# imaranresearch/LAMMPS-SPHERHARM

Hardware: NVIDIA B200
Metric: contact_pair_evals_per_s (higher is better)
Workload: dtype f64

## Files before the change

lammps-spherharm_b200/csrc/pair_split_kernels.cuh:

```cuda
#pragma once
#include "pair_kernel.cuh"

namespace shgpu {

#define SPLIT_CAP 88
#define SURV_CAP 320
#define CACHE_CAP 384

struct __align__(16) SurvRec {
  double s0, s1, s2;
  int k;
  int flag;
};

struct __align__(16) PdEntry {
  long long off;
  int cnt;
  unsigned short ntrans;
  unsigned short cnt2;
  unsigned int off2;
  unsigned short nin;
  unsigned short in[5];
};
#define PD_INLINE 5

struct __align__(16) PairHot {
  int i, j, n0, n1;
  long long off;
  int img;
  unsigned char shp_i, shp_j, pad0, pad1;
};

struct EvalPlanDev {
  int total_blocks, nshape;
  int blk_start[SH_MAX_SHAPES + 1];
  long long count[SH_MAX_SHAPES];
};

struct SplitScalars {
  unsigned long long pool_count[SH_MAX_SHAPES];
  unsigned long long in_count;
  int nbig;
  int nslow;
  int slow_counter;
  int deep_counter;
};

struct SplitArgs {
  SurvRec *pool;
  unsigned char *pool_flag;
  const long long *pool_base;
  const long long *pool_cap;
  SplitScalars *sc;
  PdEntry *pd;
  int *big_list;
  int *slow_list;
  int *inpool;
  long long in_cap;
};

struct CacheArgs {
  unsigned short *pool;
  PairHot *hot;
  unsigned long long *count;
  long long cap;
  int *overflow;
  const int *invalid;
  int enabled;
  int level;
};

__device__ __forceinline__ float fp32_margin(float t0, float t1, float t2, float ra) {
  const float sc = sqrtf(fmaf(t2, t2, fmaf(t1, t1, t0 * t0))) + ra;
  return 1.9073486e-6f * sc * sc;
}

struct NodeWindow { bool skip; float cosA, xe, se, phie; };

__device__ __forceinline__ NodeWindow make_window(const DevShape &sa, double Rb, const double *x0) {
  NodeWindow w;
  const double e0 = 2.0 * x0[0], e1 = 2.0 * x0[1], e2 = 2.0 * x0[2];
  const double D2 = e0 * e0 + e1 * e1 + e2 * e2, D = sqrt(D2);
  w.skip = D >= (sa.rmax + Rb) * (1.0 + 1e-9);
  w.cosA = -2.0f; w.xe = 1.0f; w.se = 0.0f; w.phie = 0.0f;
  if (!w.skip && D > 1e-9 * (sa.rmax + Rb)) {
    const double q = D2 - Rb * Rb;
    double rc = sa.rmin;
    if (q > 0) rc = fmin(fmax(sqrt(q), sa.rmin), sa.rmax);
    const double g = (rc * rc + q) / (2.0 * rc * D);
    w.cosA = (float)g - 3e-5f;
    if (w.cosA >= 1.0f) w.skip = true;
    w.xe = fminf(1.0f, fmaxf(-1.0f, (float)(e2 / D)));
    w.se = sqrtf(fmaxf(0.0f, 1.0f - w.xe * w.xe));
    w.phie = atan2f((float)e1, (float)e0);
    if (w.phie < 0.0f) w.phie += 6.2831853f;
  }
  return w;
}

__device__ __forceinline__ void classify_row(const DevShape &sa, const NodeWindow &w, int row, int &c0, int &ccount) {
  c0 = 0; ccount = 0;
  const int nph = sa.n_phi;
  if (row >= sa.n_theta) return;
  if (w.cosA <= -1.0f) { ccount = nph; return; }
  const float xa = sa.row_x[row];
  const float sarow = sqrtf(fmaxf(0.0f, 1.0f - xa * xa));
  const float ss = sarow * w.se, xx = xa * w.xe;
  if (xx + ss < w.cosA) return;
  const float cd = (ss > 1e-12f) ? (w.cosA - xx) / ss : -2.0f;
// ... 13 lines not shown
  int face; float ma, uu, vv;
  if (ax >= ay && ax >= az) { face = f0 > 0 ? 0 : 1; ma = ax; uu = f1; vv = f2; }
  else if (ay >= az) { face = f1 > 0 ? 2 : 3; ma = ay; uu = f0; vv = f2; }
  else { face = f2 > 0 ? 4 : 5; ma = az; uu = f0; vv = f1; }
  const float im = __fdividef(1.0f, fmaxf(ma, 1e-30f)), hn = 0.5f * (float)cn;
  const int iu = min(cn - 1, max(0, (int)((uu * im + 1.0f) * hn)));
  const int iv = min(cn - 1, max(0, (int)((vv * im + 1.0f) * hn)));
  return (face * cn + iu) * cn + iv;
}

__device__ __forceinline__ double pose_element(const PairArgs &A, int a, int b, double dd0, double dd1, double dd2, int l) {
  const int st = A.stride;
  if (l < 9) {
    const int r = l / 3, k = l - 3 * r;
    double m = A.Rs[(0 + r) * st + b] * A.Rs[(0 + k) * st + a];
    m = fma(A.Rs[(3 + r) * st + b], A.Rs[(3 + k) * st + a], m);
    m = fma(A.Rs[(6 + r) * st + b], A.Rs[(6 + k) * st + a], m);
    return m;
  } else if (l < 12) {
    const int r = l - 9;
    double tt = A.Rs[(0 + r) * st + b] * dd0;
    tt = fma(A.Rs[(3 + r) * st + b], dd1, tt);
    tt = fma(A.Rs[(6 + r) * st + b], dd2, tt);
    return tt;
  }
  const int r = l - 12;
  double hx = A.Rs[(0 + r) * st + a] * dd0;
  hx = fma(A.Rs[(3 + r) * st + a], dd1, hx);
  hx = fma(A.Rs[(6 + r) * st + a], dd2, hx);
  return -0.5 * hx;
}
__device__ __forceinline__ void pose_to_smem(const PairArgs &A, int a, int b, double dd0, double dd1, double dd2, int lane,
                                             double *pose) {
  __syncwarp();
  if (lane < 15) pose[lane] = pose_element(A, a, b, dd0, dd1, dd2, lane);
  __syncwarp();
}

__device__ __forceinline__ int exact_node_stage(const double *M, const double *t, double p0, double p1, double p2, double rmax2,
                                                double rmin2, const float2 *__restrict__ cube, int cn, int use_bounds,
                                                double &s0, double &s1, double &s2) {
  s0 = fma(M[0], p0, t[0]); s0 = fma(M[1], p1, s0); s0 = fma(M[2], p2, s0);
  s1 = fma(M[3], p0, t[1]); s1 = fma(M[4], p1, s1); s1 = fma(M[5], p2, s1);
  s2 = fma(M[6], p0, t[2]); s2 = fma(M[7], p1, s2); s2 = fma(M[8], p2, s2);
  const double rho2 = fma(s2, s2, fma(s1, s1, s0 * s0));
  if (!(rho2 < rmax2)) return -1;
  if (rho2 <= rmin2) return 2;
  if (!use_bounds) return 0;
  const float2 ul = __ldg(&cube[cube_cell((float)s0, (float)s1, (float)s2, cn)]);
  if (rho2 <= (double)ul.y) return 2;
  return rho2 < (double)ul.x ? 0 : -1;
}

template <int WPB>
__global__ void __launch_bounds__(WPB * 32) pair_cache_build_kernel(PairArgs A, CacheArgs C, const int *list, const int *nlist) {
  __shared__ unsigned short s_buf[WPB][2][CACHE_CAP];
  __shared__ double s_pose[WPB][16];
  const int lane = threadIdx.x & 31, warp = threadIdx.x >> 5;
  const int nwork = list ? *nlist : A.npairs;
  for (int w = blockIdx.x * WPB + warp; w < nwork; w += gridDim.x * WPB) {
  const int p = list ? list[w] : w;
  const int i = A.pair_i[p], j = A.pair_j[p];
  double d[3];
  pair_separation(A, p, i, j, d);
  const int shp_i = A.shape[i], shp_j = A.shape[j];
  double *pose = s_pose[warp];
  int cnt0 = 0, cnt1 = 0;
  bool over = false;
  for (int dir = 0; dir < 2 && !over; dir++) {
    const int a = dir ? j : i, b = dir ? i : j;
    const DevShape &sa = A.shapes[dir ? shp_j : shp_i];
    const DevShape &sb = A.shapes[dir ? shp_i : shp_j];
    const double sgn = dir ? -1.0 : 1.0;
    pose_to_smem(A, a, b, sgn * d[0], sgn * d[1], sgn * d[2], lane, pose);
    const double *M = pose, *t = pose + 9, *x0 = pose + 12;
    const double delta = sb.cache_delta[C.level], Rb = sb.rmax + delta;
    const NodeWindow w = make_window(sa, Rb, x0);
    const float4 *__restrict__ pf = sa.pf4;
    const float *__restrict__ cube = sb.cube_w2[C.level];
    const int cn = sb.cube_n, nph = sa.n_phi, nth = sa.n_theta;
    const float fM0 = (float)M[0], fM1 = (float)M[1], fM2 = (float)M[2], fM3 = (float)M[3], fM4 = (float)M[4],
                fM5 = (float)M[5], fM6 = (float)M[6], fM7 = (float)M[7], fM8 = (float)M[8];
    const float ft0 = (float)t[0], ft1 = (float)t[1], ft2 = (float)t[2];
    const float eps = fp32_margin(ft0, ft1, ft2, (float)sa.rmax);
    const float fR2 = (float)(Rb * Rb) + eps;
    const float fin = (float)((sb.rmin + 2.0 * delta) * (sb.rmin + 2.0 * delta)) + eps;
    unsigned short *buf = s_buf[warp][dir];
    int n = 0;
    if (!w.skip) {
      for (int rb = 0; rb < nth && !over; rb += 32) {
        int c0, ccount;
        classify_row(sa, w, rb + lane, c0, ccount);
        unsigned rows = __ballot_sync(0xffffffffu, ccount > 0);
        while (rows && !over) {
          const int rl = __ffs(rows) - 1;
          rows &= rows - 1;
          const int rc0 = __shfl_sync(0xffffffffu, c0, rl), rcount = __shfl_sync(0xffffffffu, ccount, rl);
          const int rowbase = (rb + rl) * nph;
          for (int cb = 0; cb < rcount; cb += 32) {
            const int cc = cb + lane;
            bool pass = false;
            int k = 0;
            if (cc < rcount) {
              int col = rc0 + cc;
              if (col >= nph) col -= nph;
              k = rowbase + col;
              const float4 q = __ldg(&pf[k]);
              const float f0 = fmaf(fM2, q.z, fmaf(fM1, q.y, fmaf(fM0, q.x, ft0)));
              const float f1 = fmaf(fM5, q.z, fmaf(fM4, q.y, fmaf(fM3, q.x, ft1)));
              const float f2 = fmaf(fM8, q.z, fmaf(fM7, q.y, fmaf(fM6, q.x, ft2)));
              const float r2 = fmaf(f2, f2, fmaf(f1, f1, f0 * f0));
              if (r2 < fR2) pass = (r2 < fin) || (r2 < __ldg(&cube[cube_cell(f0, f1, f2, cn)]) + eps);
            }
            const unsigned pm = __ballot_sync(0xffffffffu, pass);
            if (pm) {
              const int nnew = __popc(pm);
              if (n + nnew > CACHE_CAP) { over = true; break; }
              if (pass) buf[n + __popc(pm & ((1u << lane) - 1u))] = (unsigned short)k;
              n += nnew;
            }
          }
        }
      }
    }
    if (dir) cnt1 = n; else cnt0 = n;
    __syncwarp();
  }
  const int ntot = cnt0 + cnt1;
  long long off = 0;
  if (lane == 0 && !over && ntot > 0) off = (long long)atomicAdd(C.count, (unsigned long long)ntot);
  off = __shfl_sync(0xffffffffu, off, 0);
  if (!over && ntot > 0) {
    if (off + ntot <= C.cap) {
      for (int r = lane; r < cnt0; r += 32) C.pool[off + r] = s_buf[warp][0][r];
      for (int r = lane; r < cnt1; r += 32) C.pool[off + cnt0 + r] = s_buf[warp][1][r];
    } else { if (lane == 0) *C.overflow = 1; over = true; }
  }
  if (lane == 0) {
    PairHot hrec;
    hrec.i = i; hrec.j = j; hrec.n0 = over ? -1 : cnt0; hrec.n1 = over ? -1 : cnt1; hrec.off = off; hrec.img = A.pair_img[p];
    hrec.shp_i = (unsigned char)shp_i; hrec.shp_j = (unsigned char)shp_j; hrec.pad0 = 0; hrec.pad1 = 0;
    C.hot[p] = hrec;
  }
  __syncwarp();
  }
}

__global__ void cache_remap_kernel(PairArgs A, const int *old_half_off, const int *old_pair_j, int old_nown, const PairHot *old_hot,
                                   const unsigned short *old_pool, CacheArgs C, int *fresh_list, int *nfresh, const int *amap) {
  const int p = blockIdx.x * blockDim.x + threadIdx.x;
  const int lane = threadIdx.x & 31;
  int ntot = 0, q = -1;
  PairHot hrec;
  hrec.i = hrec.j = 0; hrec.n0 = hrec.n1 = 0; hrec.off = 0; hrec.img = 0; hrec.shp_i = hrec.shp_j = 0; hrec.pad0 = hrec.pad1 = 0;
  if (p < A.npairs) {
    const int i = A.pair_i[p], j = A.pair_j[p], img = A.pair_img[p];
    const int oi = amap ? amap[i] : i, oj = amap ? amap[j] : j;
    if (oi >= 0 && oj >= 0 && oi < old_nown && oi < oj)
      for (int e = old_half_off[oi]; e < old_half_off[oi + 1]; e++)
        if (old_pair_j[e] == oj) { q = e; break; }
    if (q >= 0) {
      hrec = old_hot[q];
      if (hrec.n0 < 0 || hrec.img != img || hrec.i != oi || hrec.j != oj) q = -1;
      hrec.i = i; hrec.j = j;
    }
    if (q >= 0) ntot = hrec.n0 + hrec.n1;
    else fresh_list[atomicAdd(nfresh, 1)] = p;
  }
  int pre = ntot;
#pragma unroll
  for (int o = 1; o < 32; o <<= 1) { const int t = __shfl_up_sync(0xffffffffu, pre, o); if (lane >= o) pre += t; }
  const int wtot = __shfl_sync(0xffffffffu, pre, 31);
  long long base = 0;
  if (lane == 31 && wtot > 0) base = (long long)atomicAdd(C.count, (unsigned long long)wtot);
  base = __shfl_sync(0xffffffffu, base, 31);
  if (q >= 0) {
    const long long off = base + (pre - ntot);
    if (off + ntot <= C.cap) {
      const unsigned short *src = old_pool + hrec.off;
      for (int r = 0; r < ntot; r++) C.pool[off + r] = src[r];
      hrec.off = off;
    } else { *C.overflow = 1; hrec.n0 = -1; hrec.n1 = -1; hrec.off = 0; }
    C.hot[p] = hrec;
  }
}

__device__ __forceinline__ void store_pd(PdEntry *dst, long long off, int cnt, int ntrans, int nin, const unsigned short *in,
                                         unsigned int off2 = 0, int cnt2 = 0) {
  PdEntry e;
  e.off = off; e.cnt = cnt; e.ntrans = (unsigned short)ntrans; e.nin = (unsigned short)nin; e.off2 = off2; e.cnt2 = (unsigned short)cnt2;
#pragma unroll
  for (int q = 0; q < PD_INLINE; q++) e.in[q] = (in && q < nin) ? in[q] : (unsigned short)0;
  *dst = e;
}

struct ShapeLite {
  const float4 *pf4; const float2 *cube_ul; const double *px, *py, *pz;
  int cube_n, pad_;
  double rmax, rmax2, rmin2;
};
struct ShapeLiteTable { ShapeLite s[SH_MAX_SHAPES]; };

template <int WPB, int LPP>
__global__ void __launch_bounds__(WPB * 32, 32 / WPB) pair_cull_cached_kernel(PairArgs A, SplitArgs S, CacheArgs C, int use_bounds,
                                                                              const __grid_constant__ ShapeLiteTable T) {
  constexpr int PPW = 32 / LPP, U = 2;
  constexpr unsigned FULLSUB = LPP == 32 ? 0xffffffffu : ((1u << LPP) - 1u);
  __shared__ double s_dpose[WPB][PPW][2][12];
  __shared__ float s_fpose[WPB][PPW][2][12];
  __shared__ unsigned short s_surv[WPB][PPW][SURV_CAP];
  __shared__ signed char s_flag[WPB][PPW][SURV_CAP];
  __shared__ unsigned short s_in[WPB][PPW][2][8];
  const int lane = threadIdx.x & 31, warp = threadIdx.x >> 5;
  const int sub = lane / LPP, sl = lane % LPP, shift = sub * LPP;
  const int p = (blockIdx.x * WPB + warp) * PPW + sub;
  if (*C.invalid) return;
  const bool inrange = p < A.npairs;
  PairHot hot;
  hot.i = hot.j = 0; hot.n0 = hot.n1 = 0; hot.off = 0; hot.img = 21; hot.shp_i = hot.shp_j = 0;
  if (inrange) {
    const int4 *hp = reinterpret_cast<const int4 *>(C.hot + p);
    const int4 h0 = __ldg(hp), h1 = __ldg(hp + 1);
    hot.i = h0.x; hot.j = h0.y; hot.n0 = h0.z; hot.n1 = h0.w;
    hot.off = (long long)(((unsigned long long)(unsigned)h1.y << 32) | (unsigned)h1.x);
    hot.img = h1.z; hot.shp_i = (unsigned char)(h1.w & 255); hot.shp_j = (unsigned char)((h1.w >> 8) & 255);
  }
  if (inrange && hot.n0 < 0 && sl == 0) S.slow_list[atomicAdd(&S.sc->nslow, 1)] = p;
  const bool cached = inrange && hot.n0 >= 0;
  const int n0 = cached ? hot.n0 : 0, n1 = cached ? hot.n1 : 0, ntot = n0 + n1;
  if (cached && ntot == 0 && sl < 2) store_pd(&S.pd[2 * p + sl], 0, 0, 0, 0, nullptr);
  const int maxtot = __reduce_max_sync(0xffffffffu, ntot);
  if (maxtot == 0) return;
  const bool work = ntot > 0;
  const int i = hot.i, j = hot.j, shp_i = hot.shp_i, shp_j = hot.shp_j;
  const ShapeLite &si = T.s[shp_i], &sj = T.s[shp_j];
  if (work) {
    const int st = A.stride;
    double d[3];
#pragma unroll
    for (int k = 0; k < 3; k++) {
      double dk = A.c[k * st + i] - A.c[k * st + j];
      const int n = ((hot.img >> (2 * k)) & 3) - 1;
      if (n != 0) dk = dk - A.boxlen[k] * (double)n;
      d[k] = dk;
    }
    if (sl < 15) {
      const int half = sl >= 12, l = half ? sl - 3 : sl;
      const double sgn = half ? -1.0 : 1.0;
      const double val = pose_element(A, half ? j : i, half ? i : j, sgn * d[0], sgn * d[1], sgn * d[2], l);
      s_dpose[warp][sub][half][l] = val;
      s_fpose[warp][sub][half][l] = (float)val;
      if (sl < 9) {
        const int r = sl / 3, k = sl - 3 * r;
        s_dpose[warp][sub][1][3 * k + r] = val;
        s_fpose[warp][sub][1][3 * k + r] = (float)val;
      }
    }
  }
  __syncwarp();
  const float4 *__restrict__ pf_i = si.pf4, *__restrict__ pf_j = sj.pf4;
  const float2 *__restrict__ cube_i = si.cube_ul, *__restrict__ cube_j = sj.cube_ul;
  const int cn_i = si.cube_n, cn_j = sj.cube_n;
  const float eps0 = fp32_margin(s_fpose[warp][sub][0][9], s_fpose[warp][sub][0][10], s_fpose[warp][sub][0][11], (float)si.rmax);
  const float eps1 = fp32_margin(s_fpose[warp][sub][1][9], s_fpose[warp][sub][1][10], s_fpose[warp][sub][1][11], (float)sj.rmax);
  const float fR20 = (float)sj.rmax2 + eps0, fR21 = (float)si.rmax2 + eps1;
  const unsigned short *__restrict__ cl = C.pool + hot.off;
  unsigned short *surv = s_surv[warp][sub];
  signed char *sflag = s_flag[warp][sub];
  int nsurv = 0, ns0 = 0;
  bool big = false;
  for (int base = 0; base < maxtot; base += LPP * U) {
    int k[U];
    float4 q[U];
    bool pass[U];
#pragma unroll
    for (int u = 0; u < U; u++) {
      const int g = base + LPP * u + sl;
      k[u] = (work && !big && g < ntot) ? (int)__ldg(&cl[g]) : -1;
    }
#pragma unroll
    for (int u = 0; u < U; u++) {
      const int dirc = (base + LPP * u + sl) >= n0;
      q[u] = k[u] >= 0 ? __ldg(&(dirc ? pf_j : pf_i)[k[u]]) : make_float4(0.f, 0.f, 0.f, 0.f);
// ... 504 lines not shown
```

lammps-spherharm_b200/csrc/shgpu_api.cu:

```cuda
#include <cuda_runtime.h>

#include <algorithm>
#include <cmath>
#include <cstdio>
#include <cstring>
#include <string>
#include <vector>

#include "../../include/shgpu.h"
#include "devbuf.h"
#include "dd_types.h"
#include "neighbor_kernels.cuh"
#include "pair_kernel.cuh"
#include "pair_warp_kernel.cuh"
#include "pair_split_kernels.cuh"
#include "shape_tables.h"
#include "step_kernels.cuh"
#include "atom_stress_kernels.cuh"

using namespace shgpu;

namespace {

struct ShapeDev {
// ... 10 lines not shown

struct sh_ctx {
  std::string err;
  int device = 0, sm_count = 148;
  cudaStream_t stream = nullptr;
  double lo[3] = {-1e30, -1e30, -1e30}, hi[3] = {1e30, 1e30, 1e30};
  int periodic[3] = {0, 0, 0};
  bool box_set = false;
  int n_theta = 32, n_phi = 64;
  std::vector<ShapeTables> shapes;
  std::vector<ShapeDev> shape_dev;
  std::vector<DevShape> shape_host_view;
  DevBuf<DevShape> d_shapes;
  bool shapes_dirty = true;
  int total_terms = 0;
  std::vector<double> pk, pm;
  std::vector<double> pgn, pgt, pmu;
  bool dissip = false;
  DevBuf<double> d_pk, d_pm, d_pgn, d_pgt, d_pmu, stress_part;
  bool coeff_dirty = true;
  WallSet walls{};
  double g[3] = {0, 0, 0}, skin = 0.0, dt = 1e-4, gamma_lin = 0.0, gamma_rot = 0.0;
  int neigh_every = 1, neigh_check = 1;
  int64_t n = 0, nghost = 0;
  int stride = 0;
  DevBuf<double> x, v, q, L, f, tq, c, Rs, c0, wallf, ewall, ke;
  DevBuf<int> shape;
  std::vector<int64_t> tag;
  DevBuf<long long> d_tag;
  bool tags_host_valid = true;
  DevBuf<double> gf;
  double time = 0.0;
  DdCtx dd;
  int *h_lagflag = nullptr;
  cudaEvent_t ev_lag[2] = {nullptr, nullptr};
  int lag_slot = 0; bool lag_pending = false, lag_mode = true, lag_pred_valid = false;
  bool cache_sync_ranks = false;
  int64_t step_index = 0, cache_build_step = -10;
  double cache_time = 0.0;
  bool step_trace = false;
  std::vector<cudaEvent_t> ev_step;
  std::vector<float> step_ms;
  std::vector<int> step_flags, step_flags_last;
  DevBuf<int> cell_of, cell_count, cell_start, cell_fill, cell_atoms, tile_sum, cnt_full, cnt_half, nbr_off, half_off,
      nbr_j, pair_i, pair_j, pair_eij, pair_eji, pair_img, scalars;
  DevBuf<double> bbox, slot, pres, stage;
  DevBuf<SurvRec> pool;
  DevBuf<unsigned char> pool_flag;
  DevBuf<long long> pool_base, pool_cap;
  DevBuf<PdEntry> pd;
  DevBuf<PairHot> cache_hot[2];
  DevBuf<SplitScalars> split_sc;
  DevBuf<EvalPlanDev> eval_plan;
  DevBuf<int> big_list, slow_list, split_flags;
  DevBuf<int> inpool;
  long long h_in_cap = 0;
  std::vector<long long> h_pool_cap;
  unsigned long long *h_pool_count = nullptr;
  SplitScalars *h_split_sc = nullptr;
  int *h_cache_invalid = nullptr;
  cudaEvent_t ev_sc = nullptr;
  bool sc_pending = false;
  int sc_nshape = 0;
  double sec_eval = 0, sec_cull = 0, sec_reduce = 0, sec_deep = 0, sec_cache = 0; int64_t eval_launches = 0;
  std::vector<int> ev2_kind;
  int64_t big_pairs = 0, slow_pairs = 0, pool_grows = 0, cache_builds = 0;
  int cache_level = 0, cache_level_pin = -1;
  int64_t cache_age = 0;
  bool cache_exhausted = false;
  int cube_n = 0;
  int reduce_occ = 0;
  int eval_pts = 0, eval_occ = 0, eval_mode = 0;
  long long last_records = 0;
  DevBuf<unsigned short> cache_pool[2];
  DevBuf<int> old_half_off, old_pair_j, fresh_list;
  int old_nown = 0, cache_cur = 0;
  DevBuf<double> old_c, old_cc0, old_cq0;
  DevBuf<long long> old_tag;
  DevBuf<int> ghost_hash, amap;
  int old_n = 0, old_stride = 0, ghost_hash_size = 0;
  bool carry = false;
  int64_t cache_remaps = 0, atoms_epoch = 0, cache_epoch = -1;
  DevBuf<unsigned long long> cache_count;
  long long cache_cap = 0;
  int cache_state = 0;
  DevBuf<double> cc0, cq0, drift;
  bool eval_pending = false;
  DevBuf<unsigned long long> counters;
  int npairs = 0, nentries = 0, nrows = 0;
  int slot_stride = 0, pres_stride = 0;
  int *h_pinned = nullptr;
  bool forces_valid = false, list_valid = false;
  int64_t steps_since_build = 0;
  int64_t neighbor_builds = 0, kernel_launches = 0;
  std::vector<cudaEvent_t> ev, ev2;
  size_t ev_used = 0, ev2_used = 0;
  double sec_pair = 0, sec_neigh = 0, sec_comm = 0, sec_other = 0, sec_run_last = 0, sec_run_total = 0;
  cudaEvent_t run_e0 = nullptr, run_e1 = nullptr;
  int64_t pair_launches = 0;
  DevBuf<double> as_vir, as_kin, as_en, as_send, as_recv;
  DevBuf<int> as_cnt, as_epair;
  int tune_threads = 0, tune_ctas_per_sm = 0, tune_variant = 0, tune_cull_wpb = 0, tune_cull_lpp = 0;
};

namespace {

int fail(sh_ctx *h, const std::string &m) { h->err = m; return -1; }
// ... 271 lines not shown
    return launch_pair_warp<16, true>(h, P, cps, max_grid);
  }
  if (tw == 256) return launch_pair_warp<8, false>(h, P, cps, max_grid);
  return launch_pair_warp<16, false>(h, P, cps, max_grid);
}

template <int WPB, int PTS, int MINB>
int launch_eval(sh_ctx *h, const SplitArgs &S, int maxT) {
  const size_t smem = (size_t)maxT * 24 + 32;
  auto kern = pair_eval_kernel<WPB, PTS, MINB>;
  CU(cudaFuncSetAttribute(kern, cudaFuncAttributeMaxDynamicSharedMemorySize, (int)std::max<size_t>(smem, 48 * 1024)));
  int occ = 0;
  CU(cudaOccupancyMaxActiveBlocksPerMultiprocessor(&occ, kern, WPB * 32, smem));
  if (occ < 1) return fail(h, "pair_eval_kernel does not fit on an SM");
  const int rpb = WPB * 32 * PTS;
  eval_plan_kernel<<<1, 32, 0, h->stream>>>(S, (int)h->shapes.size(), rpb, h->eval_plan.p);
  const int chunked = h->eval_mode == 2;
  int grid = occ * h->sm_count;
  if (!chunked) {
    long long est = h->last_records > 0 ? h->last_records + h->last_records / 16 : 0;
    if (est == 0) for (long long c : h->h_pool_cap) est += c;
    grid = (int)std::max<long long>(grid, std::min<long long>(est / rpb + (long long)h->shapes.size() + 1, 1 << 22));
  }
  kern<<<grid, WPB * 32, smem, h->stream>>>(h->d_shapes.p, S, h->eval_plan.p, h->counters.p, chunked);
  h->kernel_launches += 2;
  return 0;
}

int absorb_split_feedback(sh_ctx *h) {
  if (!h->sc_pending) return 0;
  CU(cudaEventSynchronize(h->ev_sc));
  h->sc_pending = false;
  const SplitScalars &sc = *h->h_split_sc;
  h->big_pairs += sc.nbig; h->slow_pairs += sc.nslow;
  const int ns = std::min<int>(h->sc_nshape, (int)h->h_pool_cap.size());
  for (int s = 0; s < ns; s++)
    if ((long long)sc.pool_count[s] > h->h_pool_cap[s] * 9 / 10) {
      h->h_pool_cap[s] = (long long)(sc.pool_count[s] * 3 / 2) + 4096;
      h->pool_grows++;
    }
  if ((long long)sc.in_count > h->h_in_cap * 9 / 10) { h->h_in_cap = (long long)(sc.in_count * 3 / 2) + 4096; h->pool_grows++; }
  h->last_records = 0;
  for (int s = 0; s < ns; s++) h->last_records += (long long)std::min<unsigned long long>(sc.pool_count[s], (unsigned long long)h->h_pool_cap[s]);
  if (!h->cache_sync_ranks && (h->h_cache_invalid[0] != 0 || h->h_cache_invalid[1] != 0) && h->cache_state != CACHE_INVALID) { h->cache_state = CACHE_INVALID; h->cache_exhausted = true; }
  return 0;
}

int run_split_pipeline(sh_ctx *h, PairArgs &P) {
  const int ns = (int)h->shapes.size(), np = P.npairs;
  constexpr int WPB = 8;
  int rc;
  if ((rc = absorb_split_feedback(h))) return rc;
  try {
    h->pd.ensure((size_t)2 * np + 2); h->big_list.ensure(np + 1); h->slow_list.ensure(np + 1);
    h->pool_base.ensure(SH_MAX_SHAPES); h->pool_cap.ensure(SH_MAX_SHAPES); h->split_sc.ensure(1); h->eval_plan.ensure(1); h->split_flags.ensure(4);
  } catch (std::string &e) { return fail(h, e); }
  if (!h->h_pool_count) {
    CU(cudaMallocHost(&h->h_pool_count, 8 * sizeof(unsigned long long)));
    CU(cudaMallocHost(&h->h_split_sc, sizeof(SplitScalars)));
    CU(cudaMallocHost(&h->h_cache_invalid, 2 * sizeof(int)));
    CU(cudaEventCreateWithFlags(&h->ev_sc, cudaEventDisableTiming));
  }
  if ((int)h->h_pool_cap.size() != ns) {
    h->h_pool_cap.assign(ns, std::max<long long>(4096, (long long)np * 24 / std::max(1, ns) * 2));
  }
  auto tick = [&](int kind) -> int { return ev_tick(h, kind); };
  auto tock = [&]() { ev_tock(h); };
  const int use_bounds = (h->tune_variant & 2) ? 0 : 1;
  CacheArgs C;
  C.enabled = (h->tune_variant & (8 | 2)) ? 0 : 1;
  C.invalid = h->scalars.p + 3;
  if (C.enabled) {
    const int cur = h->cache_cur;
    try { h->cache_hot[cur].ensure((size_t)np + 2); h->cache_count.ensure(2); h->fresh_list.ensure((size_t)np + 2); }
    catch (std::string &e) { return fail(h, e); }
    double pc[3];
    for (int d = 0; d < 3; d++) pc[d] = (h->hi[d] < 1e29 && h->lo[d] > -1e29) ? 0.5 * (h->lo[d] + h->hi[d]) : 0.0;
    auto check_validity = [&]() -> int {
      double dmin = 1e300;
      for (auto &sh : h->shapes) dmin = std::min(dmin, sh.cache_delta[h->cache_level]);
      double rmaxg = 0;
      for (auto &sh : h->shapes) rmaxg = std::max(rmaxg, sh.rmax);
      const double rpair = 2.0 * rmaxg + 2.0 * h->skin;
      CU(cudaMemsetAsync(h->drift.p, 0, CACHE_FIT_N * sizeof(double), h->stream));
      cache_drift_kernel<<<cdiv(h->n, 256), 256, 0, h->stream>>>(view_all(h), pc[0], pc[1], pc[2], h->drift.p);
      cache_fit_solve_kernel<<<1, 32, 0, h->stream>>>(h->drift.p, h->drift.p + 32);
      cache_check_kernel<<<cdiv(h->n, 256), 256, 0, h->stream>>>(view_all(h), h->d_shapes.p, h->cache_level, 0.5 * dmin, h->drift.p + 32,
                                                                 pc[0], pc[1], pc[2], rpair, h->scalars.p + 3);
      h->kernel_launches += 3;
      return 0;
    };
    if (h->cache_state == CACHE_REMAP && h->cache_level + 1 < SH_CACHE_LEVELS && !(h->tune_variant & 32)) {
      const int nxt = 1 - cur;
      try { h->cache_hot[nxt].ensure((size_t)np + 2); h->cache_pool[nxt].ensure((size_t)h->cache_cap + 64); }
      catch (std::string &e) { return fail(h, e); }
      const int *amap = nullptr;
      if (h->carry) {
        try { h->amap.ensure((size_t)h->n + 2); } catch (std::string &e) { return fail(h, e); }
        const int nstay = h->dd.last_nstay, nown = (int)(h->n - h->nghost);
        CU(cudaMemsetAsync(h->drift.p + 64, 0, CACHE_FIT_N * sizeof(double), h->stream));
        const double le_doff = h->dd.le_rate * h->dd.glen[1] * (h->time - h->cache_time);
        dd_cache_map_kernel<<<cdiv(h->n, 256), 256, 0, h->stream>>>(view_all(h), h->d_tag.p, nown, nstay, h->dd.order.p, h->old_tag.p, h->old_c.p,
                                                                    h->old_stride, h->old_nown, h->old_n, h->ghost_hash.p, h->ghost_hash_size,
                                                                    0.25 * h->dd.G.rc * h->dd.G.rc, h->old_cc0.p, h->old_cq0.p, h->amap.p, h->dd.glen[1], le_doff,
                                                                    pc[0], pc[1], pc[2], h->drift.p + 64);
        cache_fit_solve_kernel<<<1, 32, 0, h->stream>>>(h->drift.p + 64, h->drift.p + 96);
        dd_cache_new_atoms_kernel<<<cdiv(h->n, 256), 256, 0, h->stream>>>(view_all(h), h->amap.p, h->drift.p + 96, pc[0], pc[1], pc[2]);
// ... 11 lines not shown
                                                                h->cache_pool[cur].p, C, h->fresh_list.p, h->split_flags.p + 3, amap);
      pair_cache_build_kernel<4><<<std::max(1, std::min(cdiv(np, 4), h->sm_count * 8)), 4 * 32, 0, h->stream>>>(P, C, h->fresh_list.p, h->split_flags.p + 3);
      tock();
      h->kernel_launches += 2;
      h->cache_cur = nxt; h->cache_state = CACHE_VALID; h->cache_remaps++;
    } else if (h->cache_state != CACHE_VALID) {
      if (h->cache_level_pin >= 0) h->cache_level = h->cache_level_pin;
      else if (h->cache_exhausted) {
        if (h->cache_age < 40 && h->cache_level < 1) h->cache_level++;
        else if (h->cache_age > 400 && h->cache_level > 0) h->cache_level--;
      }
      h->cache_exhausted = false;
      if (h->cache_cap < (long long)np * 48) h->cache_cap = (long long)np * 48;
      if (tick(4)) return -2;
      for (int attempt = 0;; attempt++) {
        if (attempt > 6) return fail(h, "candidate cache kept overflowing");
        try { h->cache_pool[cur].ensure((size_t)h->cache_cap + 64); } catch (std::string &e) { return fail(h, e); }
        CU(cudaMemsetAsync(h->cache_count.p, 0, 2 * sizeof(unsigned long long), h->stream));
        CU(cudaMemsetAsync(h->split_flags.p + 2, 0, sizeof(int), h->stream));
        C.pool = h->cache_pool[cur].p; C.hot = h->cache_hot[cur].p; C.count = h->cache_count.p;
        C.cap = h->cache_cap; C.overflow = h->split_flags.p + 2; C.level = h->cache_level;
        pair_cache_build_kernel<4><<<cdiv(np, 4), 4 * 32, 0, h->stream>>>(P, C, nullptr, nullptr);
        h->kernel_launches++;
        CU(cudaMemcpyAsync(h->h_pool_count, h->cache_count.p, sizeof(unsigned long long), cudaMemcpyDeviceToHost, h->stream));
        CU(cudaMemcpyAsync(h->h_pool_count + 1, h->split_flags.p + 2, sizeof(int), cudaMemcpyDeviceToHost, h->stream));
        CU(cudaStreamSynchronize(h->stream));
        if (*reinterpret_cast<const int *>(h->h_pool_count + 1) == 0) break;
        h->cache_cap = (long long)(h->h_pool_count[0] * 3 / 2) + 4096;
      }
      cache_origin_kernel<<<cdiv(h->n, 256), 256, 0, h->stream>>>(view_all(h));
      CU(cudaMemsetAsync(h->scalars.p + 3, 0, 2 * sizeof(int), h->stream));
      tock();
      h->kernel_launches++;
      h->cache_state = CACHE_VALID; h->cache_builds++; h->cache_age = 0; h->cache_epoch = h->atoms_epoch; h->cache_build_step = h->step_index;
      h->cache_time = h->time;
    } else {
      if ((rc = check_validity())) return rc;
    }
    h->cache_age++;
  }
  C.pool = h->cache_pool[h->cache_cur].p; C.hot = h->cache_hot[h->cache_cur].p; C.count = h->cache_count.p;
  C.cap = h->cache_cap; C.overflow = h->split_flags.p + 2; C.level = h->cache_level;
  std::vector<long long> base(ns);
  long long tot = 0;
  for (int s2 = 0; s2 < ns; s2++) { base[s2] = tot; tot += h->h_pool_cap[s2]; }
  if (h->h_in_cap < (long long)np * 2 + 4096) h->h_in_cap = (long long)np * 2 + 4096;
  if (h->h_in_cap > 0xfffffff0LL) h->h_in_cap = 0xfffffff0LL;
  try { h->pool.ensure((size_t)tot + 64); h->pool_flag.ensure((size_t)tot + 64); h->inpool.ensure((size_t)h->h_in_cap + 64); } catch (std::string &e) { return fail(h, e); }
  CU(cudaMemcpyAsync(h->pool_base.p, base.data(), ns * sizeof(long long), cudaMemcpyHostToDevice, h->stream));
  CU(cudaMemcpyAsync(h->pool_cap.p, h->h_pool_cap.data(), ns * sizeof(long long), cudaMemcpyHostToDevice, h->stream));
  CU(cudaMemsetAsync(h->split_sc.p, 0, sizeof(SplitScalars), h->stream));
  SplitArgs S;
  S.pool = h->pool.p; S.pool_flag = h->pool_flag.p; S.pool_base = h->pool_base.p; S.pool_cap = h->pool_cap.p; S.sc = h->split_sc.p;
  S.pd = h->pd.p; S.big_list = h->big_list.p; S.slow_list = h->slow_list.p; S.inpool = h->inpool.p; S.in_cap = h->h_in_cap;
  if (tick(0)) return -2;
  if (C.enabled) {
    const int cw = h->tune_cull_wpb > 0 ? h->tune_cull_wpb : 1;
    const int ppw = h->tune_cull_lpp == 32 ? 1 : 2;
    const int grid = cdiv(np, cw * ppw);
    ShapeLiteTable T{};
    for (int s2 = 0; s2 < ns && s2 < SH_MAX_SHAPES; s2++) {
      const DevShape &v = h->shape_host_view[s2];
      T.s[s2].pf4 = v.pf4; T.s[s2].cube_ul = v.cube_ul; T.s[s2].px = v.px; T.s[s2].py = v.py; T.s[s2].pz = v.pz;
      T.s[s2].cube_n = v.cube_n; T.s[s2].rmax = v.rmax; T.s[s2].rmax2 = v.rmax2; T.s[s2].rmin2 = v.rmin2;
    }
#define LAUNCH_CULL(W, L) pair_cull_cached_kernel<W, L><<<grid, W * 32, 0, h->stream>>>(P, S, C, use_bounds, T)
    if (ppw == 1) { if (cw == 1) LAUNCH_CULL(1, 32); else if (cw == 2) LAUNCH_CULL(2, 32); else if (cw == 8) LAUNCH_CULL(8, 32); else LAUNCH_CULL(4, 32); }
    else { if (cw == 1) LAUNCH_CULL(1, 16); else if (cw == 2) LAUNCH_CULL(2, 16); else if (cw == 8) LAUNCH_CULL(8, 16); else LAUNCH_CULL(4, 16); }
#undef LAUNCH_CULL
    h->kernel_launches++;
  }
  {
    constexpr int WW = 2;
    const int grid = std::max(1, std::min(cdiv(np, WW), h->sm_count * 16));
    pair_cull_window_kernel<WW><<<grid, WW * 32, 0, h->stream>>>(P, S, C, use_bounds);
    h->kernel_launches++;
  }
  tock();
  int maxT = 1;
  for (int s2 = 0; s2 < ns; s2++) maxT = std::max(maxT, h->shape_host_view[s2].nterms4 + 4);
  if (tick(1)) return -2;
  if (h->eval_pts == 2) rc = h->eval_occ == 3 ? launch_eval<WPB, 2, 3>(h, S, maxT) : launch_eval<WPB, 2, 4>(h, S, maxT);
  else rc = launch_eval<WPB, 4, 2>(h, S, maxT);
  if (rc) return rc;
  tock();
  h->eval_launches++;
  if (tick(2)) return -2;
  if (h->reduce_occ == 4) pair_reduce_kernel<4><<<cdiv(np, 128), 128, 0, h->stream>>>(P, S);
  else if (h->reduce_occ == 8) pair_reduce_kernel<8><<<cdiv(np, 128), 128, 0, h->stream>>>(P, S);
  else pair_reduce_kernel<6><<<cdiv(np, 128), 128, 0, h->stream>>>(P, S);
  tock();
  h->kernel_launches++;
  {
    PairArgs Pb = P;
    Pb.pair_list = h->big_list.p; Pb.npairs = np; Pb.npairs_dev = &h->split_sc.p->nbig; Pb.work_counter = &h->split_sc.p->deep_counter;
    if (tick(3)) return -2;
    rc = launch_fused(h, Pb, h->sm_count);
    if (rc) return rc;
    tock();
    h->kernel_launches++;
  }
  CU(cudaMemcpyAsync(h->h_split_sc, h->split_sc.p, sizeof(SplitScalars), cudaMemcpyDeviceToHost, h->stream));
  CU(cudaMemcpyAsync(h->h_cache_invalid, h->scalars.p + 3, 2 * sizeof(int), cudaMemcpyDeviceToHost, h->stream));
  CU(cudaEventRecord(h->ev_sc, h->stream));
  h->sc_pending = true; h->sc_nshape = ns;
  return 0;
}

int compute_forces_device(sh_ctx *h) {
// ... 123 lines not shown
extern "C" {

int sh_version(void) { return 100; }

int sh_create(sh_ctx **out, int device_id) {
  if (!out) return -1;
  *out = nullptr;
  int ndev = 0;
  if (cudaGetDeviceCount(&ndev) != cudaSuccess || ndev == 0) return -3;
  if (device_id < 0 || device_id >= ndev) return -4;
  sh_ctx *h = new sh_ctx();
  h->device = device_id;
  if (cudaSetDevice(device_id) != cudaSuccess) { delete h; return -5; }
  cudaDeviceProp prop;
  cudaGetDeviceProperties(&prop, device_id);
  h->sm_count = prop.multiProcessorCount;
  if (cudaStreamCreateWithFlags(&h->stream, cudaStreamNonBlocking) != cudaSuccess) { delete h; return -6; }
  h->pk.assign(SH_MAX_SHAPES * SH_MAX_SHAPES, 1.0);
  h->pm.assign(SH_MAX_SHAPES * SH_MAX_SHAPES, 1.0);
  h->pgn.assign(SH_MAX_SHAPES * SH_MAX_SHAPES, 0.0); h->pgt.assign(SH_MAX_SHAPES * SH_MAX_SHAPES, 0.0); h->pmu.assign(SH_MAX_SHAPES * SH_MAX_SHAPES, 0.0);
  try {
    h->scalars.ensure(16); h->bbox.ensure(8); h->counters.ensure(16); h->drift.ensure(128);
  } catch (std::string &) { delete h; return -7; }
  cudaMemset(h->scalars.p, 0, 16 * sizeof(int));
  cudaMemset(h->counters.p, 0, 16 * sizeof(unsigned long long));
  cudaMallocHost(&h->h_pinned, 64);
  cudaMallocHost(&h->h_lagflag, 16 * sizeof(int));
  std::memset(h->h_lagflag, 0, 16 * sizeof(int));
  cudaMallocHost(&h->dd.h_int, 256 * sizeof(int));
  for (auto &e : h->ev_lag) cudaEventCreateWithFlags(&e, cudaEventDisableTiming);
  cudaEventCreate(&h->run_e0); cudaEventCreate(&h->run_e1);
  h->ev.resize(2048); h->ev2.resize(4096); h->ev2_kind.resize(2048);
  for (auto &e : h->ev) cudaEventCreate(&e);
  for (auto &e : h->ev2) cudaEventCreate(&e);
  *out = h;
  return 0;
}

int sh_destroy(sh_ctx *h) {
  if (!h) return 0;
  cudaSetDevice(h->device);
  cudaStreamSynchronize(h->stream);
  for (auto &d : h->shape_dev) { d.Ap.release(); d.ab.release(); d.node.release(); d.row_x.release(); d.cube.release(); d.pf4.release(); for (auto &w : d.cubew) w.release(); }
  h->d_shapes.release(); h->d_pk.release(); h->d_pm.release(); h->d_pgn.release(); h->d_pgt.release(); h->d_pmu.release(); h->stress_part.release();
  DevBuf<double> *db[] = {&h->x, &h->v, &h->q, &h->L, &h->f, &h->tq, &h->c, &h->Rs, &h->c0, &h->wallf, &h->ewall, &h->ke, &h->bbox, &h->slot, &h->pres};
  for (auto *b : db) b->release();
  DevBuf<int> *ib[] = {&h->shape, &h->cell_of, &h->cell_count, &h->cell_start, &h->cell_fill, &h->cell_atoms, &h->tile_sum, &h->cnt_full,
                       &h->cnt_half, &h->nbr_off, &h->half_off, &h->nbr_j, &h->pair_i, &h->pair_j, &h->pair_eij, &h->pair_eji, &h->pair_img, &h->scalars};
  for (auto *b : ib) b->release();
  h->counters.release();
  h->as_vir.release(); h->as_kin.release(); h->as_en.release(); h->as_send.release(); h->as_recv.release(); h->as_cnt.release(); h->as_epair.release();
  for (auto &e : h->ev) cudaEventDestroy(e);
  for (auto &e : h->ev2) cudaEventDestroy(e);
  h->pool.release(); h->pool_flag.release(); h->pool_base.release(); h->pool_cap.release(); h->split_sc.release(); h->eval_plan.release(); h->slow_list.release();
  h->pd.release(); h->big_list.release(); h->split_flags.release(); h->inpool.release();
  for (int k = 0; k < 2; k++) { h->cache_hot[k].release(); h->cache_pool[k].release(); }
  h->old_c.release(); h->old_cc0.release(); h->old_cq0.release(); h->old_tag.release(); h->ghost_hash.release(); h->amap.release();
  h->old_half_off.release(); h->old_pair_j.release(); h->fresh_list.release(); h->cache_count.release(); h->cc0.release(); h->cq0.release(); h->drift.release();
  if (h->h_pool_count) { cudaFreeHost(h->h_pool_count); cudaFreeHost(h->h_split_sc); cudaFreeHost(h->h_cache_invalid); cudaEventDestroy(h->ev_sc); }
  if (h->h_pinned) cudaFreeHost(h->h_pinned);
  if (h->h_lagflag) cudaFreeHost(h->h_lagflag);
  if (h->dd.h_int) cudaFreeHost(h->dd.h_int);
  for (auto &e : h->ev_lag) if (e) cudaEventDestroy(e);
  for (auto &e : h->ev_step) cudaEventDestroy(e);
  dd_peer_release(h);
  if (h->dd.peer.d_err) cudaFree(h->dd.peer.d_err);
  h->dd.peer.d_off.release();
  if (h->dd.comm && h->dd.nccl) h->dd.nccl->CommDestroy(h->dd.comm);
  {
    DdCtx &D = h->dd;
    DevBuf<int> *ib2[] = {&D.flag, &D.pos, &D.order, &D.d_int, &D.send_idx, &D.send_slot, &D.shape2};
    for (auto *b : ib2) b->release();
    DevBuf<double> *db2[] = {&D.sendbuf, &D.recvbuf, &D.x2, &D.v2, &D.q2, &D.L2, &h->gf};
    for (auto *b : db2) b->release();
    D.tag2.release(); h->d_tag.release();
  }
  h->stage.release();
  cudaEventDestroy(h->run_e0); cudaEventDestroy(h->run_e1);
  cudaStreamDestroy(h->stream);
  delete h;
  return 0;
}

const char *sh_last_error(const sh_ctx *h) { return h ? h->err.c_str() : "null handle"; }

int sh_set_box(sh_ctx *h, const double lo[3], const double hi[3], const int periodic[3]) {
  for (int d = 0; d < 3; d++) if (!(hi[d] > lo[d])) return fail(h, "box: hi <= lo");
  for (int d = 0; d < 3; d++) { h->lo[d] = lo[d]; h->hi[d] = hi[d]; h->periodic[d] = periodic[d] != 0; }
  for (int d = 0; d < 3; d++) { h->dd.glo[d] = lo[d]; h->dd.ghi[d] = hi[d]; h->dd.gper[d] = periodic[d] != 0; }
  h->dd.geometry_ok = false; h->dd.borders_ok = false;
  h->box_set = true; h->forces_valid = false; h->list_valid = false;
  return 0;
}

int sh_set_quadrature(sh_ctx *h, int n_theta, int n_phi) {
  if (!h->shapes.empty()) return fail(h, "set_quadrature must precede add_shape");
  if (n_theta < 2 || n_phi < 4) return fail(h, "quadrature too small");
  if ((long)n_theta * n_phi > 65535) return fail(h, "quadrature has more than 65535 nodes");
  h->n_theta = n_theta; h->n_phi = n_phi;
  return 0;
}

int sh_add_shape(sh_ctx *h, int lmax, const double *a_lm, const double *b_lm, double density, int *shape_id_out) try {
  if ((int)h->shapes.size() >= SH_MAX_SHAPES) return fail(h, "too many shapes");
  ShapeTables t;
  std::string e = build_shape_tables(lmax, a_lm, b_lm, density, h->n_theta, h->n_phi, t, h->cube_n);
  if (!e.empty()) return fail(h, e);
// ... 882 lines not shown
```

Baseline: 497.2 million.

## Flatten cache-build row loop into packed lane work and warp-cooperative pool copy

The cache-build kernel used to walk each candidate row separately, which left lanes idle on short rows. It now prefix-sums row counts across the warp and maps a flat index onto (row, column) with a binary search over shuffles. Two 32-wide chunks are processed per iteration so loads can overlap. The hot-record migration now copies old pool entries with the whole warp per record instead of one serial loop per lane, at the cost of extra shuffles for index decoding.

```diff
diff --git a/lammps-spherharm_b200/csrc/pair_split_kernels.cuh b/lammps-spherharm_b200/csrc/pair_split_kernels.cuh
--- a/lammps-spherharm_b200/csrc/pair_split_kernels.cuh
+++ b/lammps-spherharm_b200/csrc/pair_split_kernels.cuh
@@ -174,6 +174,7 @@
   return rho2 < (double)ul.x ? 0 : -1;
 }
 
+#define CB_U 2
 template <int WPB>
 __global__ void __launch_bounds__(WPB * 32) pair_cache_build_kernel(PairArgs A, CacheArgs C, const int *list, const int *nlist) {
   __shared__ unsigned short s_buf[WPB][2][CACHE_CAP];
@@ -213,33 +214,48 @@
       for (int rb = 0; rb < nth && !over; rb += 32) {
         int c0, ccount;
         classify_row(sa, w, rb + lane, c0, ccount);
-        unsigned rows = __ballot_sync(0xffffffffu, ccount > 0);
-        while (rows && !over) {
-          const int rl = __ffs(rows) - 1;
-          rows &= rows - 1;
-          const int rc0 = __shfl_sync(0xffffffffu, c0, rl), rcount = __shfl_sync(0xffffffffu, ccount, rl);
-          const int rowbase = (rb + rl) * nph;
-          for (int cb = 0; cb < rcount; cb += 32) {
-            const int cc = cb + lane;
-            bool pass = false;
-            int k = 0;
-            if (cc < rcount) {
-              int col = rc0 + cc;
-              if (col >= nph) col -= nph;
-              k = rowbase + col;
-              const float4 q = __ldg(&pf[k]);
-              const float f0 = fmaf(fM2, q.z, fmaf(fM1, q.y, fmaf(fM0, q.x, ft0)));
-              const float f1 = fmaf(fM5, q.z, fmaf(fM4, q.y, fmaf(fM3, q.x, ft1)));
-              const float f2 = fmaf(fM8, q.z, fmaf(fM7, q.y, fmaf(fM6, q.x, ft2)));
-              const float r2 = fmaf(f2, f2, fmaf(f1, f1, f0 * f0));
-              if (r2 < fR2) pass = (r2 < fin) || (r2 < __ldg(&cube[cube_cell(f0, f1, f2, cn)]) + eps);
-            }
-            const unsigned pm = __ballot_sync(0xffffffffu, pass);
-            if (pm) {
+        int incl = ccount;
+#pragma unroll
+        for (int o = 1; o < 32; o <<= 1) { const int t = __shfl_up_sync(0xffffffffu, incl, o); if (lane >= o) incl += t; }
+        const int excl = incl - ccount, total = __shfl_sync(0xffffffffu, incl, 31);
+        for (int fb = 0; fb < total && !over; fb += 32 * CB_U) {
+          int k[CB_U];
+          bool valid[CB_U], pass[CB_U];
+#pragma unroll
+          for (int u = 0; u < CB_U; u++) {
+            const int f = fb + 32 * u + lane;
+            int r = 0;
+#pragma unroll
+            for (int step = 16; step > 0; step >>= 1)
+              if (__shfl_sync(0xffffffffu, incl, r + step - 1) <= f) r += step;
+            const int rc0 = __shfl_sync(0xffffffffu, c0, r), rex = __shfl_sync(0xffffffffu, excl, r);
+            int col = rc0 + (f - rex);
+            if (col >= nph) col -= nph;
+            valid[u] = f < total;
+            k[u] = valid[u] ? (rb + r) * nph + col : 0;
+          }
+          float4 q[CB_U];
+#pragma unroll
+          for (int u = 0; u < CB_U; u++) q[u] = valid[u] ? __ldg(&pf[k[u]]) : make_float4(0.f, 0.f, 0.f, 0.f);
+#pragma unroll
+          for (int u = 0; u < CB_U; u++) {
+            const float f0 = fmaf(fM2, q[u].z, fmaf(fM1, q[u].y, fmaf(fM0, q[u].x, ft0)));
+            const float f1 = fmaf(fM5, q[u].z, fmaf(fM4, q[u].y, fmaf(fM3, q[u].x, ft1)));
+            const float f2 = fmaf(fM8, q[u].z, fmaf(fM7, q[u].y, fmaf(fM6, q[u].x, ft2)));
+            const float r2 = fmaf(f2, f2, fmaf(f1, f1, f0 * f0));
+            pass[u] = false;
+            if (valid[u] && r2 < fR2) pass[u] = (r2 < fin) || (r2 < __ldg(&cube[cube_cell(f0, f1, f2, cn)]) + eps);
+          }
+#pragma unroll
+          for (int u = 0; u < CB_U; u++) {
+            const unsigned pm = __ballot_sync(0xffffffffu, pass[u]);
+            if (pm && !over) {
               const int nnew = __popc(pm);
-              if (n + nnew > CACHE_CAP) { over = true; break; }
-              if (pass) buf[n + __popc(pm & ((1u << lane) - 1u))] = (unsigned short)k;
-              n += nnew;
+              if (n + nnew > CACHE_CAP) over = true;
+              else {
+                if (pass[u]) buf[n + __popc(pm & ((1u << lane) - 1u))] = (unsigned short)k[u];
+                n += nnew;
+              }
             }
           }
         }
@@ -296,14 +312,19 @@
   long long base = 0;
   if (lane == 31 && wtot > 0) base = (long long)atomicAdd(C.count, (unsigned long long)wtot);
   base = __shfl_sync(0xffffffffu, base, 31);
+  bool copy = false;
+  long long src = 0;
   if (q >= 0) {
     const long long off = base + (pre - ntot);
-    if (off + ntot <= C.cap) {
-      const unsigned short *src = old_pool + hrec.off;
-      for (int r = 0; r < ntot; r++) C.pool[off + r] = src[r];
-      hrec.off = off;
-    } else { *C.overflow = 1; hrec.n0 = -1; hrec.n1 = -1; hrec.off = 0; }
+    if (off + ntot <= C.cap) { copy = ntot > 0; src = hrec.off; hrec.off = off; }
+    else { *C.overflow = 1; hrec.n0 = -1; hrec.n1 = -1; hrec.off = 0; }
     C.hot[p] = hrec;
+  }
+  for (unsigned m = __ballot_sync(0xffffffffu, copy); m; m &= m - 1) {
+    const int l = __ffs(m) - 1;
+    const long long s0 = __shfl_sync(0xffffffffu, src, l), d0 = __shfl_sync(0xffffffffu, hrec.off, l);
+    const int n = __shfl_sync(0xffffffffu, ntot, l);
+    for (int r = lane; r < n; r += 32) C.pool[d0 + r] = old_pool[s0 + r];
   }
 }
 
```

Result: no change. 498.6 million, median of 6 (+0.3%).

## Compact cached cull pairs into a worklist before the cull kernel

Applied to the files above, without the earlier changes.

Adds a pre-pass kernel that classifies each pair: slow pairs go to the slow list, zero-count pairs get empty pd entries, and pairs with work are compacted into a cull list via warp ballot plus atomics. The cull kernel then indexes through this list and exits early for warps past the list length, so no warps are spent on empty or slow pairs. It costs an extra launch, an extra pass over the hot records and one indirection, and the grid is still sized for all pairs. The list order depends on atomics, which can reduce locality between neighbouring pairs.

```diff
diff --git a/lammps-spherharm_b200/csrc/pair_split_kernels.cuh b/lammps-spherharm_b200/csrc/pair_split_kernels.cuh
--- a/lammps-spherharm_b200/csrc/pair_split_kernels.cuh
+++ b/lammps-spherharm_b200/csrc/pair_split_kernels.cuh
@@ -44,6 +44,7 @@
   int nslow;
   int slow_counter;
   int deep_counter;
+  int ncull;
 };
 
 struct SplitArgs {
@@ -55,6 +56,7 @@
   PdEntry *pd;
   int *big_list;
   int *slow_list;
+  int *cull_list;
   int *inpool;
   long long in_cap;
 };
@@ -323,6 +325,23 @@
 };
 struct ShapeLiteTable { ShapeLite s[SH_MAX_SHAPES]; };
 
+__global__ void __launch_bounds__(256) pair_cull_list_kernel(PairArgs A, SplitArgs S, CacheArgs C) {
+  const int p = blockIdx.x * blockDim.x + threadIdx.x, lane = threadIdx.x & 31;
+  bool take = false;
+  if (p < A.npairs && !*C.invalid) {
+    const int4 h0 = __ldg(reinterpret_cast<const int4 *>(C.hot + p));
+    const int n0 = h0.z, n1 = h0.w;
+    if (n0 < 0) S.slow_list[atomicAdd(&S.sc->nslow, 1)] = p;
+    else if (n0 + n1 == 0) { store_pd(&S.pd[2 * p], 0, 0, 0, 0, nullptr); store_pd(&S.pd[2 * p + 1], 0, 0, 0, 0, nullptr); }
+    else take = true;
+  }
+  const unsigned m = __ballot_sync(0xffffffffu, take);
+  int base = 0;
+  if (lane == 0 && m) base = atomicAdd(&S.sc->ncull, __popc(m));
+  base = __shfl_sync(0xffffffffu, base, 0);
+  if (take) S.cull_list[base + __popc(m & ((1u << lane) - 1u))] = p;
+}
+
 template <int WPB, int LPP>
 __global__ void __launch_bounds__(WPB * 32, 32 / WPB) pair_cull_cached_kernel(PairArgs A, SplitArgs S, CacheArgs C, int use_bounds,
                                                                               const __grid_constant__ ShapeLiteTable T) {
@@ -335,9 +354,11 @@
   __shared__ unsigned short s_in[WPB][PPW][2][8];
   const int lane = threadIdx.x & 31, warp = threadIdx.x >> 5;
   const int sub = lane / LPP, sl = lane % LPP, shift = sub * LPP;
-  const int p = (blockIdx.x * WPB + warp) * PPW + sub;
-  if (*C.invalid) return;
-  const bool inrange = p < A.npairs;
+  const int w = (blockIdx.x * WPB + warp) * PPW + sub;
+  const int nlist = S.sc->ncull;
+  if ((blockIdx.x * WPB + warp) * PPW >= nlist) return;
+  const bool inrange = w < nlist;
+  const int p = inrange ? S.cull_list[w] : 0;
   PairHot hot;
   hot.i = hot.j = 0; hot.n0 = hot.n1 = 0; hot.off = 0; hot.img = 21; hot.shp_i = hot.shp_j = 0;
   if (inrange) {
@@ -347,10 +368,7 @@
     hot.off = (long long)(((unsigned long long)(unsigned)h1.y << 32) | (unsigned)h1.x);
     hot.img = h1.z; hot.shp_i = (unsigned char)(h1.w & 255); hot.shp_j = (unsigned char)((h1.w >> 8) & 255);
   }
-  if (inrange && hot.n0 < 0 && sl == 0) S.slow_list[atomicAdd(&S.sc->nslow, 1)] = p;
-  const bool cached = inrange && hot.n0 >= 0;
-  const int n0 = cached ? hot.n0 : 0, n1 = cached ? hot.n1 : 0, ntot = n0 + n1;
-  if (cached && ntot == 0 && sl < 2) store_pd(&S.pd[2 * p + sl], 0, 0, 0, 0, nullptr);
+  const int n0 = hot.n0, n1 = hot.n1, ntot = n0 + n1;
   const int maxtot = __reduce_max_sync(0xffffffffu, ntot);
   if (maxtot == 0) return;
   const bool work = ntot > 0;
diff --git a/lammps-spherharm_b200/csrc/shgpu_api.cu b/lammps-spherharm_b200/csrc/shgpu_api.cu
--- a/lammps-spherharm_b200/csrc/shgpu_api.cu
+++ b/lammps-spherharm_b200/csrc/shgpu_api.cu
@@ -86,7 +86,7 @@
   DevBuf<PairHot> cache_hot[2];
   DevBuf<SplitScalars> split_sc;
   DevBuf<EvalPlanDev> eval_plan;
-  DevBuf<int> big_list, slow_list, split_flags;
+  DevBuf<int> big_list, slow_list, cull_list, split_flags;
   DevBuf<int> inpool;
   long long h_in_cap = 0;
   std::vector<long long> h_pool_cap;
@@ -464,7 +464,7 @@
   int rc;
   if ((rc = absorb_split_feedback(h))) return rc;
   try {
-    h->pd.ensure((size_t)2 * np + 2); h->big_list.ensure(np + 1); h->slow_list.ensure(np + 1);
+    h->pd.ensure((size_t)2 * np + 2); h->big_list.ensure(np + 1); h->slow_list.ensure(np + 1); h->cull_list.ensure(np + 1);
     h->pool_base.ensure(SH_MAX_SHAPES); h->pool_cap.ensure(SH_MAX_SHAPES); h->split_sc.ensure(1); h->eval_plan.ensure(1); h->split_flags.ensure(4);
   } catch (std::string &e) { return fail(h, e); }
   if (!h->h_pool_count) {
@@ -582,9 +582,11 @@
   CU(cudaMemsetAsync(h->split_sc.p, 0, sizeof(SplitScalars), h->stream));
   SplitArgs S;
   S.pool = h->pool.p; S.pool_flag = h->pool_flag.p; S.pool_base = h->pool_base.p; S.pool_cap = h->pool_cap.p; S.sc = h->split_sc.p;
-  S.pd = h->pd.p; S.big_list = h->big_list.p; S.slow_list = h->slow_list.p; S.inpool = h->inpool.p; S.in_cap = h->h_in_cap;
+  S.pd = h->pd.p; S.big_list = h->big_list.p; S.slow_list = h->slow_list.p; S.cull_list = h->cull_list.p; S.inpool = h->inpool.p; S.in_cap = h->h_in_cap;
   if (tick(0)) return -2;
   if (C.enabled) {
+    pair_cull_list_kernel<<<cdiv(np, 256), 256, 0, h->stream>>>(P, S, C);
+    h->kernel_launches++;
     const int cw = h->tune_cull_wpb > 0 ? h->tune_cull_wpb : 1;
     const int ppw = h->tune_cull_lpp == 32 ? 1 : 2;
     const int grid = cdiv(np, cw * ppw);
@@ -814,7 +816,7 @@
   h->as_vir.release(); h->as_kin.release(); h->as_en.release(); h->as_send.release(); h->as_recv.release(); h->as_cnt.release(); h->as_epair.release();
   for (auto &e : h->ev) cudaEventDestroy(e);
   for (auto &e : h->ev2) cudaEventDestroy(e);
-  h->pool.release(); h->pool_flag.release(); h->pool_base.release(); h->pool_cap.release(); h->split_sc.release(); h->eval_plan.release(); h->slow_list.release();
+  h->pool.release(); h->pool_flag.release(); h->pool_base.release(); h->pool_cap.release(); h->split_sc.release(); h->eval_plan.release(); h->slow_list.release(); h->cull_list.release();
   h->pd.release(); h->big_list.release(); h->split_flags.release(); h->inpool.release();
   for (int k = 0; k < 2; k++) { h->cache_hot[k].release(); h->cache_pool[k].release(); }
   h->old_c.release(); h->old_cc0.release(); h->old_cq0.release(); h->old_tag.release(); h->ghost_hash.release(); h->amap.release();
```

New measurement: 496.5 million before, 465.8 million after (median of 6 runs). 6.2% lower.
